# PaoPaoRobot/ygz-slam

Measured on NVIDIA H100. Metric: tracked frames/sec, higher is better.
Workload: dtype u8+f32+f64

## Files before the change

ygz_slam_b200/csrc/align.cu:

```cuda
#include <algorithm>
#include <cstdlib>
#include <mutex>

#include <cooperative_groups.h>

#include "common.cuh"
#include "se3.cuh"
#include "track.cuh"

namespace ygzb {

namespace {

struct LevelImg {
    const uint8_t* d;
    int w, h, pitch;
};

__device__ __forceinline__ LevelImg level_img(const uint8_t* pyr, size_t slot_stride, int slot, const Geometry& g, int L) {
    return LevelImg{pyr + (size_t)slot * slot_stride + g.lv[L].off, g.lv[L].w, g.lv[L].h, g.lv[L].pitch};
}

__device__ void inverse3f(const float H[3][3], float inv[3][3]) {
#define COF(i, j) (H[(i + 1) % 3][(j + 1) % 3] * H[(i + 2) % 3][(j + 2) % 3] - H[(i + 1) % 3][(j + 2) % 3] * H[(i + 2) % 3][(j + 1) % 3])
// ... 289 lines not shown
    const uint8_t* has_mp;
    const double* T_ref;
    double* T_cur;
    int max_level, min_level, n_iter;
    double eps;
    int32_t* n_meas_out;
    int32_t* iters_out;
    float* ref_patch;
    float* gdx;
    float* gdy;
    double* frame_jac;
    uint8_t* visible;
    double* ws;
    void* feat_scratch;
    size_t feat_stride;
};

constexpr int kSparseCluster = 8;
constexpr int kSparseThreads = 256;
constexpr int kNormalTerms = 21 + 6 + 1;

__device__ bool ldlt_solve6(const double H[6][6], const double b[6], double x[6]) {
    double L[6][6], D[6];
    for (int i = 0; i < 6; ++i)
        for (int j = 0; j < 6; ++j) L[i][j] = 0;
    for (int j = 0; j < 6; ++j) {
        double d = H[j][j];
        for (int k = 0; k < j; ++k) d -= L[j][k] * L[j][k] * D[k];
        D[j] = d;
        if (!(fabs(d) > 0)) return false;
// ... 202 lines not shown
        if (rank == 0 && tid == 0 && a.iters_out) a.iters_out[prob * kMaxLevels + lvl] = it;
        __syncthreads();
    }
    cluster.sync();
    if (rank == 0 && tid == 0) {
        const SE3d Tref = se3_from_mat(a.T_ref + 12 * (size_t)prob);
        se3_to_mat(se3_mul(s_T, Tref), a.T_cur + 12 * (size_t)prob);
        a.n_meas_out[prob] = (int32_t)(s_last_nmeas / 16);
    }
}


constexpr int kSA2Threads = 256;
constexpr int kSA2Terms = 21 + 6 + 1;

struct SA2Feat {
    float patch[16], gdx[16], gdy[16];
    double FJ[12];
    double G[3];
    double xyz[3];
    float u, v;
    int ui, vi;
    int state;
    int pad;
};

__device__ __forceinline__ double sa2_rcp(double x) {
    double r;
    asm("rcp.approx.ftz.f64 %0, %1;" : "=d"(r) : "d"(x));
    r = fma(r, fma(-x, r, 1.0), r);
    r = fma(r, fma(-x, r, 1.0), r);
    return r;
}

__device__ bool ldlt_solve6_fast(const double H[6][6], const double b[6], double x[6]) {
    double L[6][6], D[6], rD[6];
    for (int j = 0; j < 6; ++j) {
        double d = H[j][j];
        for (int k = 0; k < j; ++k) d -= L[j][k] * L[j][k] * D[k];
// ... 15 lines not shown
        y[i] = s;
    }
    for (int i = 0; i < 6; ++i) y[i] *= rD[i];
    for (int i = 5; i >= 0; --i) {
        double s = y[i];
        for (int k = i + 1; k < 6; ++k) s -= L[k][i] * x[k];
        x[i] = s;
    }
    return true;
}

__global__ void __launch_bounds__(kSA2Threads) sparse_align2_kernel(const SparseArgs a, int feat_cap ) {
    namespace cg = cooperative_groups;
    cg::cluster_group cluster = cg::this_cluster();
    extern __shared__ __align__(16) unsigned char s_raw[];
    __shared__ double s_red[kSA2Threads / 32][kSA2Terms];
    __shared__ unsigned s_nm[kSA2Threads / 32];
    __shared__ double s_part[2][kSA2Terms + 1];
    __shared__ SE3d s_T, s_old;
    __shared__ double s_Tm[12];
    __shared__ int s_flag;
    __shared__ double s_chi2;
    __shared__ unsigned long long s_last_nmeas;

    const int rank = (int)cluster.block_rank(), C = (int)cluster.num_blocks();
    const int prob = blockIdx.x / C, tid = threadIdx.x, lane = tid & 31, warp = tid >> 5;
    const int f0 = a.offsets[prob];
    const int nf = a.n_feat ? a.n_feat[prob] : a.offsets[prob + 1] - f0;
    const long din = a.in_off ? (long)a.in_off[prob] - f0 : 0;
    const Geometry& g = a.g;
    if (nf == 0) {
        if (rank == 0 && tid == 0) a.n_meas_out[prob] = 0;
        return;
    }
    const int per = (nf + C - 1) / C;
    const int j_lo = min(nf, rank * per), nl = min(nf, j_lo + per) - j_lo;
    SA2Feat* F = nl <= feat_cap ? reinterpret_cast<SA2Feat*>(s_raw)
                                : reinterpret_cast<SA2Feat*>(static_cast<unsigned char*>(a.feat_scratch) + (size_t)prob * a.feat_stride) + j_lo;
    if (tid == 0) {
        const SE3d Tref = se3_from_mat(a.T_ref + 12 * (size_t)prob);
        s_T = se3_mul(se3_from_mat(a.T_cur + 12 * (size_t)prob), se3_inverse(Tref));
        s_chi2 = 1e10;
        s_last_nmeas = 0;
    }
    for (int j = tid; j < nl; j += kSA2Threads) {
        SA2Feat& ft = F[j];
        const long gi = f0 + j_lo + j + din;
        ft.state = 0;
        const V3d xyz = pixel2camera(a.cam, a.px[2 * gi], a.px[2 * gi + 1], a.depth[gi]);
        ft.xyz[0] = xyz.x; ft.xyz[1] = xyz.y; ft.xyz[2] = xyz.z;
        for (int k = 0; k < 16; ++k) ft.patch[k] = 0.f;
    }
    __syncthreads();
    int slot = 0;

    for (int lvl = a.max_level; lvl >= a.min_level; --lvl) {
        const LevelImg rim = level_img(a.pyr, a.slot_stride, a.ref_slot[prob], g, lvl);
        const LevelImg cim = level_img(a.pyr, a.slot_stride, a.cur_slot[prob], g, lvl);
        const float scale = 1.0f / (float)(1 << lvl);
        const double focal = (double)(float)((a.cam.fx + a.cam.fy) / 2);
        const double jscale = focal / (1 << lvl);
        for (int j = tid; j < nl; j += kSA2Threads) {
            SA2Feat& ft = F[j];
            const long gi = f0 + j_lo + j + din;
            for (int k = 0; k < 16; ++k) ft.gdx[k] = ft.gdy[k] = 0.f;
            ft.G[0] = ft.G[1] = ft.G[2] = 0.0;
            const float u_ref = (float)(a.px[2 * gi] * scale), v_ref = (float)(a.px[2 * gi + 1] * scale);
            const int ui = (int)floorf(u_ref), vi = (int)floorf(v_ref);
            if ((a.has_mp && !a.has_mp[gi]) || ui - 3 < 0 || vi - 3 < 0 || ui + 3 >= rim.w || vi + 3 >= rim.h) continue;
            ft.state |= 1;
            const double X = ft.xyz[0], Y = ft.xyz[1], zi = 1. / ft.xyz[2], zi2 = zi * zi;
            double* J = ft.FJ;
            J[0] = -zi; J[1] = 0; J[2] = X * zi2; J[3] = Y * J[2]; J[4] = -(1.0 + X * J[2]); J[5] = Y * zi;
            J[6] = 0; J[7] = -zi; J[8] = Y * zi2; J[9] = 1.0 + Y * J[8]; J[10] = -J[3]; J[11] = -X * zi;
            const float su = u_ref - (float)ui, sv = v_ref - (float)vi;
            const float wtl = (float)((1.0 - su) * (1.0 - sv)), wtr = (float)(su * (1.0 - sv)), wbl = (float)((1.0 - su) * sv), wbr = su * sv;
            const int st = rim.pitch;
            int pc = 0;
            double gxx = 0, gxy = 0, gyy = 0;
// ... 2 lines not shown
                for (int xx = 0; xx < 4; ++xx, ++p, ++pc) {
                    ft.patch[pc] = wtl * (float)p[0] + wtr * (float)p[1] + wbl * (float)p[st] + wbr * (float)p[st + 1];
                    const float dx = 0.5f * ((wtl * (float)p[1] + wtr * (float)p[2] + wbl * (float)p[st + 1] + wbr * (float)p[st + 2]) -
                                             (wtl * (float)p[-1] + wtr * (float)p[0] + wbl * (float)p[st - 1] + wbr * (float)p[st]));
                    const float dy = 0.5f * ((wtl * (float)p[st] + wtr * (float)p[1 + st] + wbl * (float)p[st * 2] + wbr * (float)p[st * 2 + 1]) -
                                             (wtl * (float)p[-st] + wtr * (float)p[1 - st] + wbl * (float)p[0] + wbr * (float)p[1]));
                    ft.gdx[pc] = dx;
                    ft.gdy[pc] = dy;
                    gxx += (double)dx * (double)dx;
                    gxy += (double)dx * (double)dy;
                    gyy += (double)dy * (double)dy;
                }
            }
            ft.G[0] = gxx; ft.G[1] = gxy; ft.G[2] = gyy;
        }
        if (tid == 0) {
            s_old = s_T;
            s_flag = 0;
            se3_to_mat(s_T, s_Tm);
        }
        __syncthreads();

        int it = 0;
        for (it = 0; it < a.n_iter; ++it) {
            for (int j = tid; j < nl; j += kSA2Threads) {
                SA2Feat& ft = F[j];
                if (!(ft.state & 1)) continue;
                ft.state &= ~2;
                const double x = s_Tm[0] * ft.xyz[0] + s_Tm[1] * ft.xyz[1] + s_Tm[2] * ft.xyz[2] + s_Tm[3];
                const double y = s_Tm[4] * ft.xyz[0] + s_Tm[5] * ft.xyz[1] + s_Tm[6] * ft.xyz[2] + s_Tm[7];
                const double z = s_Tm[8] * ft.xyz[0] + s_Tm[9] * ft.xyz[1] + s_Tm[10] * ft.xyz[2] + s_Tm[11];
                double pu, pv;
                camera2pixel(a.cam, V3d{x, y, z}, &pu, &pv);
                const float u_cur = (float)pu * scale, v_cur = (float)pv * scale;
                const int ui = (int)floorf(u_cur), vi = (int)floorf(v_cur);
                if (ui < 0 || vi < 0 || ui - 3 < 0 || vi - 3 < 0 || ui + 3 >= cim.w || vi + 3 >= cim.h) continue;
                ft.u = u_cur; ft.v = v_cur; ft.ui = ui; ft.vi = vi;
                ft.state |= 2;
            }
            __syncthreads();
            double acc[kSA2Terms];
#pragma unroll
            for (int k = 0; k < kSA2Terms; ++k) acc[k] = 0.0;
            unsigned nm = 0;
            for (int item = tid; item < nl * 4; item += kSA2Threads) {
                const SA2Feat& ft = F[item >> 2];
                if ((ft.state & 3) != 3) continue;
                const int y = item & 3;
                const float su = ft.u - (float)ft.ui, sv = ft.v - (float)ft.vi;
                const float wtl = (float)((1.0 - su) * (1.0 - sv)), wtr = (float)(su * (1.0 - sv)), wbl = (float)((1.0 - su) * sv), wbr = su * sv;
                const int st = cim.pitch;
                const uint8_t* p = cim.d + (size_t)(ft.vi + y - 2) * st + (ft.ui - 2);
                double sa = 0, sb = 0;
#pragma unroll
                for (int xx = 0; xx < 4; ++xx, ++p) {
                    const int pc = 4 * y + xx;
                    const float inten = wtl * (float)p[0] + wtr * (float)p[1] + wbl * (float)p[st] + wbr * (float)p[st + 1];
                    const float res = inten - ft.patch[pc];
                    acc[27] += (double)(res * res);
                    sa += (double)ft.gdx[pc] * (double)res;
                    sb += (double)ft.gdy[pc] * (double)res;
                }
                nm += 4;
#pragma unroll
                for (int k = 0; k < 6; ++k) acc[21 + k] -= (ft.FJ[k] * sa + ft.FJ[6 + k] * sb) * jscale;
                if (y == 0) {
                    const double s2 = jscale * jscale, gxx = ft.G[0] * s2, gxy = ft.G[1] * s2, gyy = ft.G[2] * s2;
                    int t = 0;
#pragma unroll
                    for (int r = 0; r < 6; ++r)
#pragma unroll
                        for (int c = r; c < 6; ++c, ++t)
                            acc[t] += gxx * (ft.FJ[r] * ft.FJ[c]) + gxy * (ft.FJ[r] * ft.FJ[6 + c] + ft.FJ[6 + r] * ft.FJ[c]) + gyy * (ft.FJ[6 + r] * ft.FJ[6 + c]);
                }
            }
#pragma unroll
            for (int k = 0; k < kSA2Terms; ++k) {
                double v = acc[k];
#pragma unroll
                for (int o = 16; o > 0; o >>= 1) v += __shfl_down_sync(0xFFFFFFFFu, v, o);
                if (lane == 0) s_red[warp][k] = v;
            }
#pragma unroll
            for (int o = 16; o > 0; o >>= 1) nm += __shfl_down_sync(0xFFFFFFFFu, nm, o);
            if (lane == 0) s_nm[warp] = nm;
            __syncthreads();
            if (tid <= kSA2Terms) {
                double v = 0;
                if (tid < kSA2Terms) {
                    for (int w = 0; w < kSA2Threads / 32; ++w) v += s_red[w][tid];
                } else {
                    unsigned n = 0;
                    for (int w = 0; w < kSA2Threads / 32; ++w) n += s_nm[w];
                    v = (double)n;
                }
                s_part[slot][tid] = v;
            }
            cluster.sync();
            if (tid == 0) {
                double tot[kSA2Terms];
                unsigned long long n_meas = 0;
                for (int k = 0; k < kSA2Terms; ++k) tot[k] = 0;
                for (int r = 0; r < C; ++r) {
                    const double* pr = cluster.map_shared_rank(&s_part[slot][0], r);
                    for (int k = 0; k < kSA2Terms; ++k) tot[k] += pr[k];
                    n_meas += (unsigned long long)pr[kSA2Terms];
                }
                s_last_nmeas = n_meas;
                double H[6][6], b[6], x[6];
                int t = 0;
                for (int r = 0; r < 6; ++r)
                    for (int c = r; c < 6; ++c) H[r][c] = H[c][r] = tot[t++];
                for (int k = 0; k < 6; ++k) b[k] = tot[21 + k];
                const double new_chi2 = (double)((float)tot[27] / (float)n_meas);
                bool stop = !ldlt_solve6_fast(H, b, x) || isnan(x[0]);
                if ((it > 0 && new_chi2 > s_chi2) || stop) {
                    s_T = s_old;
                    s_flag = 1;
                } else {
                    double mx[6];
                    for (int k = 0; k < 6; ++k) mx[k] = -x[k];
                    const SE3d Tn = se3_mul(s_T, se3_exp(mx));
                    s_old = s_T;
                    s_T = Tn;
                    s_chi2 = new_chi2;
                    double nmx = -1;
                    for (int k = 0; k < 6; ++k) nmx = fabs(x[k]) > nmx ? fabs(x[k]) : nmx;
                    if (nmx <= a.eps) s_flag = 1;
                }
                se3_to_mat(s_T, s_Tm);
            }
            slot ^= 1;
            __syncthreads();
            if (s_flag) break;
        }
        if (rank == 0 && tid == 0 && a.iters_out) a.iters_out[prob * kMaxLevels + lvl] = it;
        __syncthreads();
    }
    cluster.sync();
    if (rank == 0 && tid == 0) {
        const SE3d Tref = se3_from_mat(a.T_ref + 12 * (size_t)prob);
        se3_to_mat(se3_mul(s_T, Tref), a.T_cur + 12 * (size_t)prob);
        a.n_meas_out[prob] = (int32_t)(s_last_nmeas / 16);
    }
}

__device__ __forceinline__ void mat34_mul(const double* A, const double* B, double* C) {
    for (int r = 0; r < 3; ++r) {
        for (int c = 0; c < 3; ++c) C[4 * r + c] = A[4 * r] * B[c] + A[4 * r + 1] * B[4 + c] + A[4 * r + 2] * B[8 + c];
        C[4 * r + 3] = A[4 * r] * B[3] + A[4 * r + 1] * B[7] + A[4 * r + 2] * B[11] + A[4 * r + 3];
    }
}
__device__ __forceinline__ void mat34_inv(const double* A, double* C) {
    for (int r = 0; r < 3; ++r) {
        for (int c = 0; c < 3; ++c) C[4 * r + c] = A[4 * c + r];
        C[4 * r + 3] = -(A[r] * A[3] + A[4 + r] * A[7] + A[8 + r] * A[11]);
    }
}
// ... 125 lines not shown
            b.c_px[2 * dst] = b.cand_px[2 * ((size_t)j * b.cap + c)];
            b.c_px[2 * dst + 1] = b.cand_px[2 * ((size_t)j * b.cap + c) + 1];
            b.c_pw[3 * dst] = st.kf_pw[3 * fe];
            b.c_pw[3 * dst + 1] = st.kf_pw[3 * fe + 1];
            b.c_pw[3 * dst + 2] = st.kf_pw[3 * fe + 2];
        }
        __syncthreads();
        if (tid == 0) s_carry += chunk_total;
        __syncthreads();
    }
    if (tid == 0) b.c_cnt[j] = s_carry;
}

}

size_t sparse_align2_scratch_bytes(int n_problems, int max_features) { return (size_t)n_problems * max_features * sizeof(SA2Feat); }
size_t sparse_align_ws_doubles(int n_problems) { return (size_t)n_problems * 2 * kSparseCluster * (kNormalTerms + 1); }

int launch_align2d(ygzb_frames* f, int n, const int32_t* d_slot, const uint8_t* d_level, const uint8_t* d_ref_border,
                   const uint8_t* d_ref, int n_iter, double* d_uv, uint8_t* d_ok) {
    ygzb_ctx* ctx = f->ctx;
    if (n <= 0) return YGZB_OK;
    ProfScope ps(ctx, kStageAlign2D);
    align2d_kernel<<<(n + 127) / 128, 128, 0, ctx->stream>>>(f->d_pyr, ctx->slot_stride, ctx->geo, n, d_slot, d_level, d_ref_border,
                                                             d_ref, n_iter, d_uv, d_ok);
    YGZB_LAUNCHED(ctx);
    return YGZB_OK;
}

int launch_align1d(ygzb_frames* f, int n, const int32_t* d_slot, const uint8_t* d_level, const float* d_dir, const uint8_t* d_ref_border,
                   const uint8_t* d_ref, int n_iter, double* d_uv, uint8_t* d_ok, double* d_hinv) {
// ... 29 lines not shown
    cfg.dynamicSmemBytes = 0;
    cfg.stream = ctx->stream;
    cudaLaunchAttribute attr[1];
    attr[0].id = cudaLaunchAttributeClusterDimension;
    attr[0].val.clusterDim.x = cluster;
    attr[0].val.clusterDim.y = 1;
    attr[0].val.clusterDim.z = 1;
    cfg.attrs = attr;
    cfg.numAttrs = 1;
    ProfScope ps(ctx, kStageSparseAlign);
    YGZB_CUDA(ctx, cudaLaunchKernelEx(&cfg, sparse_align_kernel, a));
    YGZB_LAUNCHED(ctx);
    return YGZB_OK;
}

int launch_sparse_align2(ygzb_ctx* ctx, SparseArgs a, int n_problems, int cluster, void* feat_scratch, size_t feat_stride) {
    static std::once_flag once;
    static int max_dyn = 0;
    std::call_once(once, [&] {
        int dev = 0, optin = 0;
        cudaGetDevice(&dev);
        cudaDeviceGetAttribute(&optin, cudaDevAttrMaxSharedMemoryPerBlockOptin, dev);
        max_dyn = optin - 8 * 1024;
        cudaFuncSetAttribute(sparse_align2_kernel, cudaFuncAttributeMaxDynamicSharedMemorySize, max_dyn);
    });
    const int max_features = (int)(feat_stride / sizeof(SA2Feat));
    const int feat_cap = std::min(max_dyn / (int)sizeof(SA2Feat), (max_features + cluster - 1) / cluster);
    a.feat_scratch = feat_scratch;
    a.feat_stride = feat_stride;
    cudaLaunchConfig_t cfg{};
    cfg.gridDim = dim3((unsigned)(n_problems * cluster));
    cfg.blockDim = dim3(kSA2Threads);
    cfg.dynamicSmemBytes = (size_t)feat_cap * sizeof(SA2Feat);
    cfg.stream = ctx->stream;
    cudaLaunchAttribute attr[1];
    attr[0].id = cudaLaunchAttributeClusterDimension;
    attr[0].val.clusterDim.x = cluster;
    attr[0].val.clusterDim.y = 1;
    attr[0].val.clusterDim.z = 1;
    cfg.attrs = attr;
    cfg.numAttrs = 1;
    ProfScope ps(ctx, kStageSparseAlign);
    YGZB_CUDA(ctx, cudaLaunchKernelEx(&cfg, sparse_align2_kernel, a, feat_cap));
    YGZB_LAUNCHED(ctx);
    return YGZB_OK;
}

}
// ... 24 lines not shown
    a.T_cur = d_T_cur;
    a.max_level = max_level;
    a.min_level = min_level;
    a.n_iter = n_iter;
    a.eps = eps;
    a.n_meas_out = d_n_meas;
    a.iters_out = d_iters;
    a.ref_patch = d_ref_patch;
    a.gdx = d_gdx;
    a.gdy = d_gdy;
    a.frame_jac = d_frame_jac;
    a.visible = d_visible;
    a.ws = d_ws;
    a.feat_scratch = nullptr;
    a.feat_stride = 0;
    if (sparse_align_gen1()) return launch_sparse_align1(ctx, a, n_problems, kSparseCluster);
    return launch_sparse_align2(ctx, a, n_problems, kTrackCluster, d_feat_scratch, feat_stride);
}


int launch_track_chain_front(ygzb_frames* f, const TrackStore& st, const TrackBatch& b, int sparse_cluster) {
    ygzb_ctx* ctx = f->ctx;
    if (b.J <= 0) return YGZB_OK;
    {
        ProfScope ps(ctx, kStageOther);
        track_prep_kernel<<<(b.J + 127) / 128, 128, 0, ctx->stream>>>(st, b);
        YGZB_LAUNCHED(ctx);
    }
    const bool gen1 = sparse_align_gen1();
    if (gen1)
        YGZB_CUDA(ctx, cudaMemsetAsync(b.ref_patch, 0, (size_t)b.J * st.cells * 16 * sizeof(float), ctx->stream));
    SparseArgs a;
// ... 13 lines not shown
    a.T_cur = b.T_cur;
    a.max_level = 2;
    a.min_level = 0;
    a.n_iter = 30;
    a.eps = 1e-6;
    a.n_meas_out = b.n_meas;
    a.iters_out = nullptr;
    a.ref_patch = b.ref_patch;
    a.gdx = b.gdx;
    a.gdy = b.gdy;
    a.frame_jac = b.frame_jac;
    a.visible = b.visible;
    a.ws = b.sparse_ws;
    a.feat_scratch = nullptr;
    a.feat_stride = 0;
    if (gen1) return launch_sparse_align1(ctx, a, b.J, sparse_cluster);
    return launch_sparse_align2(ctx, a, b.J, sparse_cluster, b.sa2_scratch, sparse_align2_scratch_bytes(1, st.cells));
}

int launch_track_chain_mid(ygzb_frames* f, const TrackStore& st, const TrackBatch& b) {
    ygzb_ctx* ctx = f->ctx;
    if (b.J <= 0) return YGZB_OK;
    {
        ProfScope ps(ctx, kStageOther);
        track_compose_kernel<<<(b.J + 63) / 64, 64, 0, ctx->stream>>>(st, b);
        YGZB_LAUNCHED(ctx);
    }
    {
        ProfScope ps(ctx, kStageOther);
        track_motion_kernel<<<(b.J + 63) / 64, 64, 0, ctx->stream>>>(st, b);
        YGZB_LAUNCHED(ctx);
    }
// ... 17 lines not shown
```

ygz_slam_b200/csrc/common.cuh:

```cuda
#pragma once

#include <cuda_runtime.h>
#include <stdint.h>
#include <stdio.h>
#include <string.h>

#include <vector>

#include "../../include/ygz_b200.h"

namespace ygzb {

constexpr int kMaxLevels = YGZB_MAX_LEVELS;

constexpr int kTileW = 80;
constexpr int kTileH = 40;

struct LevelGeom {
    int w, h, pitch;
    unsigned off;
};

struct Geometry {
    LevelGeom lv[kMaxLevels];
// ... 121 lines not shown
                   const uint8_t* d_ref, int n_iter, double* d_uv, uint8_t* d_ok);
int launch_align1d(ygzb_frames* f, int n, const int32_t* d_slot, const uint8_t* d_level, const float* d_dir, const uint8_t* d_ref_border,
                   const uint8_t* d_ref, int n_iter, double* d_uv, uint8_t* d_ok, double* d_hinv);
int launch_project_align(ygzb_frames* f, int n, const int32_t* d_ref_slot, const int32_t* d_cur_slot, const double* d_poses,
                         const int32_t* d_ref_pose, const int32_t* d_cur_pose, const double* d_ref_px, const double* d_ref_depth,
                         const uint8_t* d_ref_level, double* d_cur_px, uint8_t* d_search_level, uint8_t* d_ok);
int launch_sparse_align(ygzb_frames* f, int n_problems, const int32_t* d_ref_slot, const int32_t* d_cur_slot,
                        const int32_t* d_offsets, const double* d_px, const double* d_depth, const uint8_t* d_has_mp,
                        const double* d_T_ref, double* d_T_cur, int max_level, int min_level, int n_iter, double eps,
                        int32_t* d_n_meas, int32_t* d_iters, float* d_ref_patch, float* d_gdx, float* d_gdy, double* d_frame_jac,
                        uint8_t* d_visible, double* d_ws, void* d_feat_scratch, size_t feat_stride);
bool sparse_align_gen1();
size_t sparse_align_ws_doubles(int n_problems);
size_t sparse_align2_scratch_bytes(int n_problems, int max_features);
constexpr int kTrackCluster = 4;

struct Carver {
    uint8_t* base;
    size_t off = 0;
    explicit Carver(void* p) : base(static_cast<uint8_t*>(p)) {}
    template <typename T>
    T* take(size_t count) {
        off = (off + 255) & ~(size_t)255;
        T* r = base ? reinterpret_cast<T*>(base + off) : nullptr;
        off += count * sizeof(T);
        return r;
    }
    size_t bytes() const { return off + 256; }
};

// ... 40 lines not shown
```

ygz_slam_b200/csrc/track.cu:

```cuda
#include <algorithm>
#include <cstdlib>
#include <cstring>
#include <new>

#include "ba2.cuh"
#include "common.cuh"
#include "se3.cuh"
#include "track.cuh"

using namespace ygzb;

struct ygzb_tracker {
    ygzb_frames* f;
    ygzb_ctx* ctx;
    TrackStore st;
    TrackBatch b;
    int max_jobs;
    void* d_store;
    void* d_batch;
    double* d_depth;
    ygzb_track_job* h_jobs;
    ygzb_keyframe_job* h_kfjobs;
    ygzb_keyframe_job* d_kfjobs;
    ygzb_keyframe_result* d_kfres;
    cudaEvent_t staged;
    int last_J;
    void* d_ba;
    size_t ba_bytes;
    int pcap, ocap;
    cudaStream_t front;
    cudaEvent_t e_fill;
    cudaEvent_t e_front;
    cudaEvent_t e_up;
    cudaEvent_t e_main;
    int cluster;
    void* d_xfer;
};

namespace {

template <typename T>
int dalloc(ygzb_ctx* ctx, T** p, size_t count) {
    return check_cuda(ctx, cudaMalloc((void**)p, std::max(count, (size_t)1) * sizeof(T)), "cudaMalloc");
}

__device__ __forceinline__ void mat34_inv(const double* A, double* C) {
    for (int r = 0; r < 3; ++r) {
        for (int c = 0; c < 3; ++c) C[4 * r + c] = A[4 * c + r];
        C[4 * r + 3] = -(A[r] * A[3] + A[4 + r] * A[7] + A[8 + r] * A[11]);
    }
}
// ... 417 lines not shown
    *out = nullptr;
    ygzb_ctx* ctx = f->ctx;
    cudaSetDevice(ctx->device);
    if (ctx->geo.n_cells > 4096) return set_error(ctx, YGZB_ERR_CAPACITY, "tracker: %d grid cells (the BA assembly handles up to 4096)", ctx->geo.n_cells);
    ygzb_tracker* t = new (std::nothrow) ygzb_tracker();
    if (!t) return YGZB_ERR_INVALID;
    memset(t, 0, sizeof(*t));
    t->f = f;
    t->ctx = ctx;
    t->max_jobs = max_jobs;
    t->cluster = kTrackCluster;
    if (const char* e = getenv("YGZB_TRACK_CLUSTER")) {
        const int v = atoi(e);
        if (v == 1 || v == 2 || v == 4 || v == 8) t->cluster = v;
    }
    const Geometry& g = ctx->geo;
    const size_t S = (size_t)n_streams, R = YGZB_TRACK_RING, cells = (size_t)g.n_cells, E = S * R, cap = kTrackMaxLocal * cells;
    TrackStore& st = t->st;
    st.S = n_streams; st.R = (int)R; st.cells = (int)cells; st.W = g.W; st.H = g.H;
    st.fx = K[0]; st.fy = K[1]; st.cx = K[2]; st.cy = K[3];
    int rc = YGZB_OK;
    {
        Carver sz(nullptr);
        sz.take<double>(E * 12); sz.take<int32_t>(E); sz.take<int32_t>(E); sz.take<long long>(E); sz.take<double>(E * cells * 2);
        sz.take<uint8_t>(E * cells); sz.take<double>(E * cells); sz.take<double>(E * cells * 3); sz.take<int32_t>(E);
        sz.take<long long>(E * cap); sz.take<double>(E * cap * 2);
        rc = check_cuda(ctx, cudaMalloc(&t->d_store, sz.bytes()), "cudaMalloc(tracker store)");
        if (rc == YGZB_OK) rc = check_cuda(ctx, cudaMemsetAsync(t->d_store, 0, sz.bytes(), ctx->stream), "memset");
        if (rc == YGZB_OK) {
            Carver c(t->d_store);
            st.kf_T = c.take<double>(E * 12); st.kf_n = c.take<int32_t>(E); st.kf_slot = c.take<int32_t>(E); st.kf_mp0 = c.take<long long>(E);
            st.kf_px = c.take<double>(E * cells * 2); st.kf_level = c.take<uint8_t>(E * cells); st.kf_depth = c.take<double>(E * cells);
            st.kf_pw = c.take<double>(E * cells * 3); st.kf_nobs = c.take<int32_t>(E); st.kf_obs_id = c.take<long long>(E * cap);
            st.kf_obs_px = c.take<double>(E * cap * 2);
        }
    }
    if (rc == YGZB_OK) rc = dalloc(ctx, &t->d_depth, S * g.W * g.H);
    st.depth_map = t->d_depth;
    if (rc == YGZB_OK) {
        const size_t J = (size_t)max_jobs, F = J * cells, Cn = J * cap;
        TrackBatch& b = t->b;
        b.J = 0;
        b.cap = (int)cap;
        auto carve = [&](Carver& c) {
            b.jobs = c.take<ygzb_track_job>(J);
            b.ref_slot = c.take<int32_t>(J); b.cur_slot = c.take<int32_t>(J); b.offsets = c.take<int32_t>(J + 1); b.in_off = c.take<int32_t>(J);
            b.n_feat = c.take<int32_t>(J); b.n_meas = c.take<int32_t>(J);
            b.T_ref = c.take<double>(J * 12); b.T_cur = c.take<double>(J * 12); b.T_aligned = c.take<double>(J * 12);
            b.ref_patch = c.take<float>(F * 16); b.gdx = c.take<float>(F * 16); b.gdy = c.take<float>(F * 16);
            b.frame_jac = c.take<double>(F * 12); b.visible = c.take<uint8_t>(F);
            b.sparse_ws = c.take<double>(sparse_align_ws_doubles((int)J));
            b.sa2_scratch = c.take<double>(sparse_align2_scratch_bytes((int)J, (int)cells) / 8 + 1);
            b.aligned = c.take<int32_t>(J); b.rel = c.take<double>(J * kTrackMaxLocal * 12);
            b.cand_ok = c.take<uint8_t>(Cn); b.cand_px = c.take<double>(Cn * 2); b.n_cand = c.take<int32_t>(J);
            b.c_cnt = c.take<int32_t>(J); b.c_off = c.take<int32_t>(J + 1); b.c_src = c.take<int32_t>(Cn);
            b.c_pw = c.take<double>(Cn * 3); b.c_px = c.take<double>(Cn * 2); b.c_depth = c.take<double>(Cn);
            b.inlier = c.take<uint8_t>(Cn); b.enable = c.take<uint8_t>(Cn); b.n_inl = c.take<int32_t>(J);
            b.pose_ws = c.take<double>(pose_only_ws_doubles((int)J));
            b.results = c.take<ygzb_track_result>(J);
        };
        Carver sz(nullptr);
        carve(sz);
        rc = check_cuda(ctx, cudaMalloc(&t->d_batch, sz.bytes()), "cudaMalloc(tracker batch)");
        if (rc == YGZB_OK) rc = check_cuda(ctx, cudaMemsetAsync(t->d_batch, 0, sz.bytes(), ctx->stream), "memset");
        if (rc == YGZB_OK) {
            Carver c(t->d_batch);
            carve(c);
        }
    }
    if (rc == YGZB_OK) rc = check_cuda(ctx, cudaMallocHost((void**)&t->h_jobs, sizeof(ygzb_track_job) * (size_t)max_jobs), "cudaMallocHost");
    if (rc == YGZB_OK) rc = check_cuda(ctx, cudaMallocHost((void**)&t->h_kfjobs, sizeof(ygzb_keyframe_job) * S), "cudaMallocHost");
    if (rc == YGZB_OK) rc = dalloc(ctx, &t->d_kfjobs, S);
    if (rc == YGZB_OK) rc = dalloc(ctx, &t->d_kfres, S);
    if (rc == YGZB_OK) rc = check_cuda(ctx, cudaMemsetAsync(t->d_kfres, 0, sizeof(ygzb_keyframe_result) * S, ctx->stream), "memset");
    if (rc == YGZB_OK) rc = check_cuda(ctx, cudaEventCreateWithFlags(&t->staged, cudaEventDisableTiming), "cudaEventCreate");
    if (rc == YGZB_OK) rc = check_cuda(ctx, cudaStreamCreateWithFlags(&t->front, cudaStreamNonBlocking), "cudaStreamCreate");
    for (cudaEvent_t* e : {&t->e_fill, &t->e_front, &t->e_main, &t->e_up})
        if (rc == YGZB_OK) rc = check_cuda(ctx, cudaEventCreateWithFlags(e, cudaEventDisableTiming), "cudaEventCreate");
    if (rc == YGZB_OK) {
        rc = check_cuda(ctx, cudaEventRecord(t->e_fill, ctx->stream), "cudaEventRecord");
        if (rc == YGZB_OK) rc = check_cuda(ctx, cudaEventRecord(t->e_main, ctx->stream), "cudaEventRecord");
        if (rc == YGZB_OK) rc = check_cuda(ctx, cudaEventRecord(t->e_up, ctx->stream), "cudaEventRecord");
    }
    if (rc == YGZB_OK) {
        t->pcap = (int)(kTrackMaxLocal * cells + 1);
// ... 10 lines not shown
        ygzb_tracker_destroy(t);
        return rc;
    }
    *out = t;
    return YGZB_OK;
}

void ygzb_tracker_destroy(ygzb_tracker* t) {
    if (!t) return;
    cudaSetDevice(t->ctx->device);
    cudaStreamSynchronize(t->ctx->stream);
    if (t->d_store) cudaFree(t->d_store);
    if (t->d_batch) cudaFree(t->d_batch);
    if (t->d_depth) cudaFree(t->d_depth);
    if (t->h_jobs) cudaFreeHost(t->h_jobs);
    if (t->h_kfjobs) cudaFreeHost(t->h_kfjobs);
    if (t->d_kfjobs) cudaFree(t->d_kfjobs);
    if (t->d_kfres) cudaFree(t->d_kfres);
    if (t->d_ba) cudaFree(t->d_ba);
    if (t->d_xfer) cudaFree(t->d_xfer);
    if (t->staged) cudaEventDestroy(t->staged);
    if (t->front) {
        cudaStreamSynchronize(t->front);
        cudaStreamDestroy(t->front);
    }
    for (cudaEvent_t e : {t->e_fill, t->e_front, t->e_main, t->e_up})
        if (e) cudaEventDestroy(e);
    delete t;
}

// ... 25 lines not shown
    if (n_jobs == 0) return YGZB_OK;
    ygzb_ctx* ctx = t->ctx;
    cudaSetDevice(ctx->device);
    if (n_jobs > t->max_jobs) return set_error(ctx, YGZB_ERR_CAPACITY, "%d jobs exceed the tracker's max_jobs %d", n_jobs, t->max_jobs);
    for (int j = 0; j < n_jobs; ++j) {
        const ygzb_track_job& q = jobs[j];
        if (q.stream < 0 || q.stream >= t->st.S || q.cur_slot < 0 || q.cur_slot >= t->f->capacity || q.n_local < 1 || q.n_local > kTrackMaxLocal - 1)
            return set_error(ctx, YGZB_ERR_INVALID, "track job %d: stream / slot / n_local out of range", j);
        for (int k = 0; k < q.n_local; ++k)
            if (q.entry[k] < 0 || q.entry[k] >= YGZB_TRACK_RING) return set_error(ctx, YGZB_ERR_INVALID, "track job %d: ring entry out of range", j);
    }
    YGZB_CUDA(ctx, cudaEventSynchronize(t->staged));
    memcpy(t->h_jobs, jobs, sizeof(ygzb_track_job) * (size_t)n_jobs);
    TrackBatch b = t->b;
    b.J = n_jobs;
    t->last_J = n_jobs;
    const int cl = t->cluster;
    int rc;
    {
        cudaStream_t main = ctx->stream;
        YGZB_CUDA(ctx, cudaStreamWaitEvent(t->front, t->e_fill, 0));
        YGZB_CUDA(ctx, cudaStreamWaitEvent(t->front, t->e_main, 0));
        ctx->stream = t->front;
        cudaError_t ce = cudaMemcpyAsync(const_cast<ygzb_track_job*>(t->b.jobs), t->h_jobs, sizeof(ygzb_track_job) * (size_t)n_jobs,
                                         cudaMemcpyHostToDevice, ctx->stream);
        if (ce == cudaSuccess) ce = cudaEventRecord(t->staged, ctx->stream);
        rc = ce == cudaSuccess ? launch_track_chain_front(t->f, t->st, b, cl) : check_cuda(ctx, ce, "H2D(track jobs)");
        if (rc == YGZB_OK) rc = check_cuda(ctx, cudaEventRecord(t->e_front, ctx->stream), "cudaEventRecord");
        ctx->stream = main;
        if (rc != YGZB_OK) return rc;
        YGZB_CUDA(ctx, cudaStreamWaitEvent(ctx->stream, t->e_front, 0));
    }
    rc = launch_track_chain_mid(t->f, t->st, b);
    if (rc != YGZB_OK) return rc;
    rc = launch_pose_only_dev(ctx, n_jobs, b.c_off, b.c_cnt, b.c_pw, b.c_px, b.T_cur, b.inlier, b.c_depth, b.n_inl, b.enable, b.pose_ws, cl, b.cap);
    if (rc != YGZB_OK) return rc;
    {
        ProfScope ps(ctx, kStageOther);
        track_finish_kernel<<<(n_jobs + 63) / 64, 64, 0, ctx->stream>>>(b);
        YGZB_LAUNCHED(ctx);
// ... 242 lines not shown
```

ygz_slam_b200/csrc/track.cuh:

```cuda
#pragma once

#include <stdint.h>

#include "../../include/ygz_b200.h"

struct ygzb_frames;

namespace ygzb {

constexpr int kTrackMaxLocal = 4;

struct TrackStore {
    int S, R, cells, W, H;
    double fx, fy, cx, cy;
    double* kf_T;
    int32_t* kf_n;
    int32_t* kf_slot;
    long long* kf_mp0;
    double* kf_px;
    uint8_t* kf_level;
    double* kf_depth;
    double* kf_pw;
    int32_t* kf_nobs;
    long long* kf_obs_id;
// ... 1 lines not shown
    const double* depth_map;
};

struct TrackBatch {
    int J;
    int cap;
    const ygzb_track_job* jobs;
    int32_t *ref_slot, *cur_slot, *offsets, *in_off, *n_feat, *n_meas;
    double *T_ref, *T_cur;
    double* T_aligned;
    float *ref_patch, *gdx, *gdy;
    double* frame_jac;
    uint8_t* visible;
    double* sparse_ws;
    void* sa2_scratch;
    int32_t* aligned;
    double* rel;
    uint8_t* cand_ok;
    double* cand_px;
    int32_t* n_cand;
    int32_t *c_cnt, *c_off;
    int32_t* c_src;
    double *c_pw, *c_px, *c_depth;
    uint8_t *inlier, *enable;
    int32_t* n_inl;
    double* pose_ws;
    ygzb_track_result* results;
};

int launch_track_chain_front(ygzb_frames* f, const TrackStore& st, const TrackBatch& b, int sparse_cluster);
// ... 8 lines not shown
```

Baseline: 29200.

## Batch sparse-alignment jobs sharing a reference frame into one cluster group

Consecutive track jobs that share the same reference keyframe entry are grouped, up to a configurable size with a default of 2. Each group is solved by a single cluster that builds the reference patches, gradients and Jacobians once and runs per-frame Gauss-Newton state side by side. The feature struct is split into a shared reference part and a per-frame current-projection part. This cuts redundant reference-side work and the number of launched clusters, but the per-frame reductions run serially inside the block, shared-memory use grows, and a group keeps iterating until its slowest frame converges.

```diff
diff --git a/ygz_slam_b200/csrc/align.cu b/ygz_slam_b200/csrc/align.cu
--- a/ygz_slam_b200/csrc/align.cu
+++ b/ygz_slam_b200/csrc/align.cu
@@ -327,6 +327,7 @@
     double* ws;
     void* feat_scratch;
     size_t feat_stride;
+    const int32_t* groups;
 };
 
 constexpr int kSparseCluster = 8;
@@ -559,15 +560,17 @@
 constexpr int kSA2Threads = 256;
 constexpr int kSA2Terms = 21 + 6 + 1;
 
-struct SA2Feat {
+struct SA2Ref {
     float patch[16], gdx[16], gdy[16];
     double FJ[12];
     double G[3];
     double xyz[3];
+    int state;
+    int pad;
+};
+struct SA2Cur {
     float u, v;
     int ui, vi;
-    int state;
-    int pad;
 };
 
 __device__ __forceinline__ double sa2_rcp(double x) {
@@ -613,38 +616,53 @@
     namespace cg = cooperative_groups;
     cg::cluster_group cluster = cg::this_cluster();
     extern __shared__ __align__(16) unsigned char s_raw[];
-    __shared__ double s_red[kSA2Threads / 32][kSA2Terms];
-    __shared__ unsigned s_nm[kSA2Threads / 32];
-    __shared__ double s_part[2][kSA2Terms + 1];
-    __shared__ SE3d s_T, s_old;
-    __shared__ double s_Tm[12];
-    __shared__ int s_flag;
-    __shared__ double s_chi2;
-    __shared__ unsigned long long s_last_nmeas;
+    __shared__ double s_red[kSA2MaxGroup][kSA2Threads / 32][kSA2Terms];
+    __shared__ unsigned s_nm[kSA2MaxGroup][kSA2Threads / 32];
+    __shared__ double s_part[2][kSA2MaxGroup][kSA2Terms + 1];
+    __shared__ SE3d s_T[kSA2MaxGroup], s_old[kSA2MaxGroup];
+    __shared__ double s_Tm[kSA2MaxGroup][12];
+    __shared__ int s_flag[kSA2MaxGroup];
+    __shared__ int s_iters[kSA2MaxGroup];
+    __shared__ double s_chi2[kSA2MaxGroup];
+    __shared__ unsigned long long s_last_nmeas[kSA2MaxGroup];
 
     const int rank = (int)cluster.block_rank(), C = (int)cluster.num_blocks();
-    const int prob = blockIdx.x / C, tid = threadIdx.x, lane = tid & 31, warp = tid >> 5;
-    const int f0 = a.offsets[prob];
-    const int nf = a.n_feat ? a.n_feat[prob] : a.offsets[prob + 1] - f0;
-    const long din = a.in_off ? (long)a.in_off[prob] - f0 : 0;
+    const int grp = blockIdx.x / C, tid = threadIdx.x, lane = tid & 31, warp = tid >> 5;
+    const int p0 = a.groups ? a.groups[2 * grp] : grp, G = a.groups ? a.groups[2 * grp + 1] : 1;
+    const int f0 = a.offsets[p0];
+    const int nf = a.n_feat ? a.n_feat[p0] : a.offsets[p0 + 1] - f0;
+    const long in0 = a.in_off ? (long)a.in_off[p0] : f0;
     const Geometry& g = a.g;
     if (nf == 0) {
-        if (rank == 0 && tid == 0) a.n_meas_out[prob] = 0;
+        if (rank == 0 && tid < G) a.n_meas_out[p0 + tid] = 0;
         return;
     }
     const int per = (nf + C - 1) / C;
     const int j_lo = min(nf, rank * per), nl = min(nf, j_lo + per) - j_lo;
-    SA2Feat* F = nl <= feat_cap ? reinterpret_cast<SA2Feat*>(s_raw)
-                                : reinterpret_cast<SA2Feat*>(static_cast<unsigned char*>(a.feat_scratch) + (size_t)prob * a.feat_stride) + j_lo;
-    if (tid == 0) {
-        const SE3d Tref = se3_from_mat(a.T_ref + 12 * (size_t)prob);
-        s_T = se3_mul(se3_from_mat(a.T_cur + 12 * (size_t)prob), se3_inverse(Tref));
-        s_chi2 = 1e10;
-        s_last_nmeas = 0;
+    SA2Ref* F;
+    unsigned char* cur_base;
+    size_t cur_stride;
+    if (nl <= feat_cap) {
+        F = reinterpret_cast<SA2Ref*>(s_raw);
+        cur_base = s_raw + (size_t)nl * sizeof(SA2Ref);
+        cur_stride = (size_t)nl * sizeof(SA2Cur);
+    } else {
+        unsigned char* base = static_cast<unsigned char*>(a.feat_scratch) + (size_t)p0 * a.feat_stride;
+        const size_t max_f = a.feat_stride / (sizeof(SA2Ref) + sizeof(SA2Cur));
+        F = reinterpret_cast<SA2Ref*>(base) + j_lo;
+        cur_base = base + max_f * sizeof(SA2Ref) + (size_t)j_lo * sizeof(SA2Cur);
+        cur_stride = a.feat_stride;
+    }
+    auto CU = [&](int fr) { return reinterpret_cast<SA2Cur*>(cur_base + (size_t)fr * cur_stride); };
+    if (tid < G) {
+        const SE3d Tref = se3_from_mat(a.T_ref + 12 * (size_t)(p0 + tid));
+        s_T[tid] = se3_mul(se3_from_mat(a.T_cur + 12 * (size_t)(p0 + tid)), se3_inverse(Tref));
+        s_chi2[tid] = 1e10;
+        s_last_nmeas[tid] = 0;
     }
     for (int j = tid; j < nl; j += kSA2Threads) {
-        SA2Feat& ft = F[j];
-        const long gi = f0 + j_lo + j + din;
+        SA2Ref& ft = F[j];
+        const long gi = in0 + j_lo + j;
         ft.state = 0;
         const V3d xyz = pixel2camera(a.cam, a.px[2 * gi], a.px[2 * gi + 1], a.depth[gi]);
         ft.xyz[0] = xyz.x; ft.xyz[1] = xyz.y; ft.xyz[2] = xyz.z;
@@ -654,14 +672,13 @@
     int slot = 0;
 
     for (int lvl = a.max_level; lvl >= a.min_level; --lvl) {
-        const LevelImg rim = level_img(a.pyr, a.slot_stride, a.ref_slot[prob], g, lvl);
-        const LevelImg cim = level_img(a.pyr, a.slot_stride, a.cur_slot[prob], g, lvl);
+        const LevelImg rim = level_img(a.pyr, a.slot_stride, a.ref_slot[p0], g, lvl);
         const float scale = 1.0f / (float)(1 << lvl);
         const double focal = (double)(float)((a.cam.fx + a.cam.fy) / 2);
         const double jscale = focal / (1 << lvl);
         for (int j = tid; j < nl; j += kSA2Threads) {
-            SA2Feat& ft = F[j];
-            const long gi = f0 + j_lo + j + din;
+            SA2Ref& ft = F[j];
+            const long gi = in0 + j_lo + j;
             for (int k = 0; k < 16; ++k) ft.gdx[k] = ft.gdy[k] = 0.f;
             ft.G[0] = ft.G[1] = ft.G[2] = 0.0;
             const float u_ref = (float)(a.px[2 * gi] * scale), v_ref = (float)(a.px[2 * gi + 1] * scale);
@@ -694,99 +711,113 @@
             }
             ft.G[0] = gxx; ft.G[1] = gxy; ft.G[2] = gyy;
         }
-        if (tid == 0) {
-            s_old = s_T;
-            s_flag = 0;
-            se3_to_mat(s_T, s_Tm);
+        if (tid < G) {
+            s_old[tid] = s_T[tid];
+            s_flag[tid] = 0;
+            s_iters[tid] = a.n_iter;
+            se3_to_mat(s_T[tid], s_Tm[tid]);
         }
         __syncthreads();
 
-        int it = 0;
-        for (it = 0; it < a.n_iter; ++it) {
-            for (int j = tid; j < nl; j += kSA2Threads) {
-                SA2Feat& ft = F[j];
-                if (!(ft.state & 1)) continue;
-                ft.state &= ~2;
-                const double x = s_Tm[0] * ft.xyz[0] + s_Tm[1] * ft.xyz[1] + s_Tm[2] * ft.xyz[2] + s_Tm[3];
-                const double y = s_Tm[4] * ft.xyz[0] + s_Tm[5] * ft.xyz[1] + s_Tm[6] * ft.xyz[2] + s_Tm[7];
-                const double z = s_Tm[8] * ft.xyz[0] + s_Tm[9] * ft.xyz[1] + s_Tm[10] * ft.xyz[2] + s_Tm[11];
+        for (int it = 0; it < a.n_iter; ++it) {
+            for (int q = tid; q < G * nl; q += kSA2Threads) {
+                const int fr = q / nl, j = q - fr * nl;
+                const SA2Ref& ft = F[j];
+                if (s_flag[fr] || !(ft.state & 1)) continue;
+                SA2Cur& cu = CU(fr)[j];
+                const double* Tm = s_Tm[fr];
+                cu.ui = -1;
+                const double x = Tm[0] * ft.xyz[0] + Tm[1] * ft.xyz[1] + Tm[2] * ft.xyz[2] + Tm[3];
+                const double y = Tm[4] * ft.xyz[0] + Tm[5] * ft.xyz[1] + Tm[6] * ft.xyz[2] + Tm[7];
+                const double z = Tm[8] * ft.xyz[0] + Tm[9] * ft.xyz[1] + Tm[10] * ft.xyz[2] + Tm[11];
                 double pu, pv;
                 camera2pixel(a.cam, V3d{x, y, z}, &pu, &pv);
                 const float u_cur = (float)pu * scale, v_cur = (float)pv * scale;
                 const int ui = (int)floorf(u_cur), vi = (int)floorf(v_cur);
+                const LevelImg cim = level_img(a.pyr, a.slot_stride, a.cur_slot[p0 + fr], g, lvl);
                 if (ui < 0 || vi < 0 || ui - 3 < 0 || vi - 3 < 0 || ui + 3 >= cim.w || vi + 3 >= cim.h) continue;
-                ft.u = u_cur; ft.v = v_cur; ft.ui = ui; ft.vi = vi;
-                ft.state |= 2;
+                cu.u = u_cur; cu.v = v_cur; cu.ui = ui; cu.vi = vi;
             }
             __syncthreads();
-            double acc[kSA2Terms];
-#pragma unroll
-            for (int k = 0; k < kSA2Terms; ++k) acc[k] = 0.0;
-            unsigned nm = 0;
-            for (int item = tid; item < nl * 4; item += kSA2Threads) {
-                const SA2Feat& ft = F[item >> 2];
-                if ((ft.state & 3) != 3) continue;
-                const int y = item & 3;
-                const float su = ft.u - (float)ft.ui, sv = ft.v - (float)ft.vi;
-                const float wtl = (float)((1.0 - su) * (1.0 - sv)), wtr = (float)(su * (1.0 - sv)), wbl = (float)((1.0 - su) * sv), wbr = su * sv;
-                const int st = cim.pitch;
-                const uint8_t* p = cim.d + (size_t)(ft.vi + y - 2) * st + (ft.ui - 2);
-                double sa = 0, sb = 0;
-#pragma unroll
-                for (int xx = 0; xx < 4; ++xx, ++p) {
-                    const int pc = 4 * y + xx;
-                    const float inten = wtl * (float)p[0] + wtr * (float)p[1] + wbl * (float)p[st] + wbr * (float)p[st + 1];
-                    const float res = inten - ft.patch[pc];
-                    acc[27] += (double)(res * res);
-                    sa += (double)ft.gdx[pc] * (double)res;
-                    sb += (double)ft.gdy[pc] * (double)res;
+#pragma unroll 1
+            for (int fr = 0; fr < G; ++fr) {
+                if (s_flag[fr]) continue;
+                const LevelImg cim = level_img(a.pyr, a.slot_stride, a.cur_slot[p0 + fr], g, lvl);
+                const SA2Cur* cur = CU(fr);
+                double acc[kSA2Terms];
+#pragma unroll
+                for (int k = 0; k < kSA2Terms; ++k) acc[k] = 0.0;
+                unsigned nm = 0;
+                for (int item = tid; item < nl * 4; item += kSA2Threads) {
+                    const SA2Ref& ft = F[item >> 2];
+                    if (!(ft.state & 1)) continue;
+                    const SA2Cur cu = cur[item >> 2];
+                    if (cu.ui < 0) continue;
+                    const int y = item & 3;
+                    const float su = cu.u - (float)cu.ui, sv = cu.v - (float)cu.vi;
+                    const float wtl = (float)((1.0 - su) * (1.0 - sv)), wtr = (float)(su * (1.0 - sv)), wbl = (float)((1.0 - su) * sv), wbr = su * sv;
+                    const int st = cim.pitch;
+                    const uint8_t* p = cim.d + (size_t)(cu.vi + y - 2) * st + (cu.ui - 2);
+                    double sa = 0, sb = 0;
+#pragma unroll
+                    for (int xx = 0; xx < 4; ++xx, ++p) {
+                        const int pc = 4 * y + xx;
+                        const float inten = wtl * (float)p[0] + wtr * (float)p[1] + wbl * (float)p[st] + wbr * (float)p[st + 1];
+                        const float res = inten - ft.patch[pc];
+                        acc[27] += (double)(res * res);
+                        sa += (double)ft.gdx[pc] * (double)res;
+                        sb += (double)ft.gdy[pc] * (double)res;
+                    }
+                    nm += 4;
+#pragma unroll
+                    for (int k = 0; k < 6; ++k) acc[21 + k] -= (ft.FJ[k] * sa + ft.FJ[6 + k] * sb) * jscale;
+                    if (y == 0) {
+                        const double s2 = jscale * jscale, gxx = ft.G[0] * s2, gxy = ft.G[1] * s2, gyy = ft.G[2] * s2;
+                        int t = 0;
+#pragma unroll
+                        for (int r = 0; r < 6; ++r)
+#pragma unroll
+                            for (int c = r; c < 6; ++c, ++t)
+                                acc[t] += gxx * (ft.FJ[r] * ft.FJ[c]) + gxy * (ft.FJ[r] * ft.FJ[6 + c] + ft.FJ[6 + r] * ft.FJ[c]) + gyy * (ft.FJ[6 + r] * ft.FJ[6 + c]);
+                    }
                 }
-                nm += 4;
-#pragma unroll
-                for (int k = 0; k < 6; ++k) acc[21 + k] -= (ft.FJ[k] * sa + ft.FJ[6 + k] * sb) * jscale;
-                if (y == 0) {
-                    const double s2 = jscale * jscale, gxx = ft.G[0] * s2, gxy = ft.G[1] * s2, gyy = ft.G[2] * s2;
-                    int t = 0;
-#pragma unroll
-                    for (int r = 0; r < 6; ++r)
-#pragma unroll
-                        for (int c = r; c < 6; ++c, ++t)
-                            acc[t] += gxx * (ft.FJ[r] * ft.FJ[c]) + gxy * (ft.FJ[r] * ft.FJ[6 + c] + ft.FJ[6 + r] * ft.FJ[c]) + gyy * (ft.FJ[6 + r] * ft.FJ[6 + c]);
+#pragma unroll
+                for (int k = 0; k < kSA2Terms; ++k) {
+                    double v = acc[k];
+#pragma unroll
+                    for (int o = 16; o > 0; o >>= 1) v += __shfl_down_sync(0xFFFFFFFFu, v, o);
+                    if (lane == 0) s_red[fr][warp][k] = v;
                 }
+#pragma unroll
+                for (int o = 16; o > 0; o >>= 1) nm += __shfl_down_sync(0xFFFFFFFFu, nm, o);
+                if (lane == 0) s_nm[fr][warp] = nm;
             }
-#pragma unroll
-            for (int k = 0; k < kSA2Terms; ++k) {
-                double v = acc[k];
-#pragma unroll
-                for (int o = 16; o > 0; o >>= 1) v += __shfl_down_sync(0xFFFFFFFFu, v, o);
-                if (lane == 0) s_red[warp][k] = v;
-            }
-#pragma unroll
-            for (int o = 16; o > 0; o >>= 1) nm += __shfl_down_sync(0xFFFFFFFFu, nm, o);
-            if (lane == 0) s_nm[warp] = nm;
             __syncthreads();
-            if (tid <= kSA2Terms) {
+            for (int q = tid; q < G * (kSA2Terms + 1); q += kSA2Threads) {
+                const int fr = q / (kSA2Terms + 1), k = q - fr * (kSA2Terms + 1);
+                if (s_flag[fr]) continue;
                 double v = 0;
-                if (tid < kSA2Terms) {
-                    for (int w = 0; w < kSA2Threads / 32; ++w) v += s_red[w][tid];
+                if (k < kSA2Terms) {
+                    for (int w = 0; w < kSA2Threads / 32; ++w) v += s_red[fr][w][k];
                 } else {
                     unsigned n = 0;
-                    for (int w = 0; w < kSA2Threads / 32; ++w) n += s_nm[w];
+                    for (int w = 0; w < kSA2Threads / 32; ++w) n += s_nm[fr][w];
                     v = (double)n;
                 }
-                s_part[slot][tid] = v;
+                s_part[slot][fr][k] = v;
             }
             cluster.sync();
-            if (tid == 0) {
+            if (tid < G && !s_flag[tid]) {
+                const int fr = tid;
                 double tot[kSA2Terms];
                 unsigned long long n_meas = 0;
                 for (int k = 0; k < kSA2Terms; ++k) tot[k] = 0;
                 for (int r = 0; r < C; ++r) {
-                    const double* pr = cluster.map_shared_rank(&s_part[slot][0], r);
+                    const double* pr = cluster.map_shared_rank(&s_part[slot][fr][0], r);
                     for (int k = 0; k < kSA2Terms; ++k) tot[k] += pr[k];
                     n_meas += (unsigned long long)pr[kSA2Terms];
                 }
-                s_last_nmeas = n_meas;
+                s_last_nmeas[fr] = n_meas;
                 double H[6][6], b[6], x[6];
                 int t = 0;
                 for (int r = 0; r < 6; ++r)
@@ -794,34 +825,41 @@
                 for (int k = 0; k < 6; ++k) b[k] = tot[21 + k];
                 const double new_chi2 = (double)((float)tot[27] / (float)n_meas);
                 bool stop = !ldlt_solve6_fast(H, b, x) || isnan(x[0]);
-                if ((it > 0 && new_chi2 > s_chi2) || stop) {
-                    s_T = s_old;
-                    s_flag = 1;
+                bool done = false;
+                if ((it > 0 && new_chi2 > s_chi2[fr]) || stop) {
+                    s_T[fr] = s_old[fr];
+                    done = true;
                 } else {
                     double mx[6];
                     for (int k = 0; k < 6; ++k) mx[k] = -x[k];
-                    const SE3d Tn = se3_mul(s_T, se3_exp(mx));
-                    s_old = s_T;
-                    s_T = Tn;
-                    s_chi2 = new_chi2;
+                    const SE3d Tn = se3_mul(s_T[fr], se3_exp(mx));
+                    s_old[fr] = s_T[fr];
+                    s_T[fr] = Tn;
+                    s_chi2[fr] = new_chi2;
                     double nmx = -1;
                     for (int k = 0; k < 6; ++k) nmx = fabs(x[k]) > nmx ? fabs(x[k]) : nmx;
-                    if (nmx <= a.eps) s_flag = 1;
+                    if (nmx <= a.eps) done = true;
                 }
-                se3_to_mat(s_T, s_Tm);
+                se3_to_mat(s_T[fr], s_Tm[fr]);
+                if (done) {
+                    s_flag[fr] = 1;
+                    s_iters[fr] = it;
+                }
             }
             slot ^= 1;
             __syncthreads();
-            if (s_flag) break;
-        }
-        if (rank == 0 && tid == 0 && a.iters_out) a.iters_out[prob * kMaxLevels + lvl] = it;
+            int active = 0;
+            for (int fr = 0; fr < G; ++fr) active |= !s_flag[fr];
+            if (!active) break;
+        }
+        if (rank == 0 && tid < G && a.iters_out) a.iters_out[(p0 + tid) * kMaxLevels + lvl] = s_iters[tid];
         __syncthreads();
     }
     cluster.sync();
-    if (rank == 0 && tid == 0) {
-        const SE3d Tref = se3_from_mat(a.T_ref + 12 * (size_t)prob);
-        se3_to_mat(se3_mul(s_T, Tref), a.T_cur + 12 * (size_t)prob);
-        a.n_meas_out[prob] = (int32_t)(s_last_nmeas / 16);
+    if (rank == 0 && tid < G) {
+        const SE3d Tref = se3_from_mat(a.T_ref + 12 * (size_t)(p0 + tid));
+        se3_to_mat(se3_mul(s_T[tid], Tref), a.T_cur + 12 * (size_t)(p0 + tid));
+        a.n_meas_out[p0 + tid] = (int32_t)(s_last_nmeas[tid] / 16);
     }
 }
 
@@ -977,7 +1015,9 @@
 
 }
 
-size_t sparse_align2_scratch_bytes(int n_problems, int max_features) { return (size_t)n_problems * max_features * sizeof(SA2Feat); }
+size_t sparse_align2_scratch_bytes(int n_problems, int max_features) {
+    return (size_t)n_problems * max_features * (sizeof(SA2Ref) + sizeof(SA2Cur));
+}
 size_t sparse_align_ws_doubles(int n_problems) { return (size_t)n_problems * 2 * kSparseCluster * (kNormalTerms + 1); }
 
 int launch_align2d(ygzb_frames* f, int n, const int32_t* d_slot, const uint8_t* d_level, const uint8_t* d_ref_border,
@@ -1037,24 +1077,28 @@
     return YGZB_OK;
 }
 
-int launch_sparse_align2(ygzb_ctx* ctx, SparseArgs a, int n_problems, int cluster, void* feat_scratch, size_t feat_stride) {
+int launch_sparse_align2(ygzb_ctx* ctx, SparseArgs a, int n_groups, int group_max, int cluster, void* feat_scratch, size_t feat_stride) {
     static std::once_flag once;
     static int max_dyn = 0;
     std::call_once(once, [&] {
         int dev = 0, optin = 0;
         cudaGetDevice(&dev);
         cudaDeviceGetAttribute(&optin, cudaDevAttrMaxSharedMemoryPerBlockOptin, dev);
-        max_dyn = optin - 8 * 1024;
+        cudaFuncAttributes fa{};
+        cudaFuncGetAttributes(&fa, sparse_align2_kernel);
+        max_dyn = optin - (int)fa.sharedSizeBytes;
         cudaFuncSetAttribute(sparse_align2_kernel, cudaFuncAttributeMaxDynamicSharedMemorySize, max_dyn);
     });
-    const int max_features = (int)(feat_stride / sizeof(SA2Feat));
-    const int feat_cap = std::min(max_dyn / (int)sizeof(SA2Feat), (max_features + cluster - 1) / cluster);
+    if (group_max < 1 || group_max > kSA2MaxGroup) return set_error(ctx, YGZB_ERR_INVALID, "sparse alignment: %d frames per group", group_max);
+    const int feat_bytes = (int)(sizeof(SA2Ref) + (size_t)group_max * sizeof(SA2Cur));
+    const int max_features = (int)(feat_stride / (sizeof(SA2Ref) + sizeof(SA2Cur)));
+    const int feat_cap = std::min(max_dyn / feat_bytes, (max_features + cluster - 1) / cluster);
     a.feat_scratch = feat_scratch;
     a.feat_stride = feat_stride;
     cudaLaunchConfig_t cfg{};
-    cfg.gridDim = dim3((unsigned)(n_problems * cluster));
+    cfg.gridDim = dim3((unsigned)(n_groups * cluster));
     cfg.blockDim = dim3(kSA2Threads);
-    cfg.dynamicSmemBytes = (size_t)feat_cap * sizeof(SA2Feat);
+    cfg.dynamicSmemBytes = (size_t)feat_cap * feat_bytes;
     cfg.stream = ctx->stream;
     cudaLaunchAttribute attr[1];
     attr[0].id = cudaLaunchAttributeClusterDimension;
@@ -1109,8 +1153,9 @@
     a.ws = d_ws;
     a.feat_scratch = nullptr;
     a.feat_stride = 0;
+    a.groups = nullptr;
     if (sparse_align_gen1()) return launch_sparse_align1(ctx, a, n_problems, kSparseCluster);
-    return launch_sparse_align2(ctx, a, n_problems, kTrackCluster, d_feat_scratch, feat_stride);
+    return launch_sparse_align2(ctx, a, n_problems, 1, kTrackCluster, d_feat_scratch, feat_stride);
 }
 
 
@@ -1154,8 +1199,9 @@
     a.ws = b.sparse_ws;
     a.feat_scratch = nullptr;
     a.feat_stride = 0;
+    a.groups = b.groups;
     if (gen1) return launch_sparse_align1(ctx, a, b.J, sparse_cluster);
-    return launch_sparse_align2(ctx, a, b.J, sparse_cluster, b.sa2_scratch, sparse_align2_scratch_bytes(1, st.cells));
+    return launch_sparse_align2(ctx, a, b.n_groups, b.group_max, sparse_cluster, b.sa2_scratch, sparse_align2_scratch_bytes(1, st.cells));
 }
 
 int launch_track_chain_mid(ygzb_frames* f, const TrackStore& st, const TrackBatch& b) {
diff --git a/ygz_slam_b200/csrc/common.cuh b/ygz_slam_b200/csrc/common.cuh
--- a/ygz_slam_b200/csrc/common.cuh
+++ b/ygz_slam_b200/csrc/common.cuh
@@ -159,6 +159,7 @@
 size_t sparse_align_ws_doubles(int n_problems);
 size_t sparse_align2_scratch_bytes(int n_problems, int max_features);
 constexpr int kTrackCluster = 4;
+constexpr int kSA2MaxGroup = 8;
 
 struct Carver {
     uint8_t* base;
diff --git a/ygz_slam_b200/csrc/track.cu b/ygz_slam_b200/csrc/track.cu
--- a/ygz_slam_b200/csrc/track.cu
+++ b/ygz_slam_b200/csrc/track.cu
@@ -35,6 +35,8 @@
     cudaEvent_t e_main;
     int cluster;
     void* d_xfer;
+    int sparse_group;
+    int32_t* h_groups;
 };
 
 namespace {
@@ -482,6 +484,11 @@
         const int v = atoi(e);
         if (v == 1 || v == 2 || v == 4 || v == 8) t->cluster = v;
     }
+    t->sparse_group = 2;
+    if (const char* e = getenv("YGZB_SPARSE_GROUP")) {
+        const int v = atoi(e);
+        if (v >= 1 && v <= kSA2MaxGroup) t->sparse_group = v;
+    }
     const Geometry& g = ctx->geo;
     const size_t S = (size_t)n_streams, R = YGZB_TRACK_RING, cells = (size_t)g.n_cells, E = S * R, cap = kTrackMaxLocal * cells;
     TrackStore& st = t->st;
@@ -512,6 +519,7 @@
         b.cap = (int)cap;
         auto carve = [&](Carver& c) {
             b.jobs = c.take<ygzb_track_job>(J);
+            b.groups = c.take<int32_t>(J * 2);
             b.ref_slot = c.take<int32_t>(J); b.cur_slot = c.take<int32_t>(J); b.offsets = c.take<int32_t>(J + 1); b.in_off = c.take<int32_t>(J);
             b.n_feat = c.take<int32_t>(J); b.n_meas = c.take<int32_t>(J);
             b.T_ref = c.take<double>(J * 12); b.T_cur = c.take<double>(J * 12); b.T_aligned = c.take<double>(J * 12);
@@ -537,6 +545,7 @@
         }
     }
     if (rc == YGZB_OK) rc = check_cuda(ctx, cudaMallocHost((void**)&t->h_jobs, sizeof(ygzb_track_job) * (size_t)max_jobs), "cudaMallocHost");
+    if (rc == YGZB_OK) rc = check_cuda(ctx, cudaMallocHost((void**)&t->h_groups, sizeof(int32_t) * 2 * (size_t)max_jobs), "cudaMallocHost");
     if (rc == YGZB_OK) rc = check_cuda(ctx, cudaMallocHost((void**)&t->h_kfjobs, sizeof(ygzb_keyframe_job) * S), "cudaMallocHost");
     if (rc == YGZB_OK) rc = dalloc(ctx, &t->d_kfjobs, S);
     if (rc == YGZB_OK) rc = dalloc(ctx, &t->d_kfres, S);
@@ -577,6 +586,7 @@
     if (t->d_batch) cudaFree(t->d_batch);
     if (t->d_depth) cudaFree(t->d_depth);
     if (t->h_jobs) cudaFreeHost(t->h_jobs);
+    if (t->h_groups) cudaFreeHost(t->h_groups);
     if (t->h_kfjobs) cudaFreeHost(t->h_kfjobs);
     if (t->d_kfjobs) cudaFree(t->d_kfjobs);
     if (t->d_kfres) cudaFree(t->d_kfres);
@@ -632,6 +642,21 @@
     memcpy(t->h_jobs, jobs, sizeof(ygzb_track_job) * (size_t)n_jobs);
     TrackBatch b = t->b;
     b.J = n_jobs;
+    b.n_groups = 0;
+    b.group_max = 0;
+    for (int j = 0, e_prev = -1; j < n_jobs; ++j) {
+        const int e = jobs[j].stream * t->st.R + jobs[j].entry[jobs[j].n_local - 1];
+        int32_t* last = t->h_groups + 2 * (b.n_groups - 1);
+        if (b.n_groups && e == e_prev && last[1] < t->sparse_group) {
+            ++last[1];
+        } else {
+            t->h_groups[2 * b.n_groups] = j;
+            t->h_groups[2 * b.n_groups + 1] = 1;
+            ++b.n_groups;
+        }
+        b.group_max = std::max(b.group_max, t->h_groups[2 * b.n_groups - 1]);
+        e_prev = e;
+    }
     t->last_J = n_jobs;
     const int cl = t->cluster;
     int rc;
@@ -642,6 +667,8 @@
         ctx->stream = t->front;
         cudaError_t ce = cudaMemcpyAsync(const_cast<ygzb_track_job*>(t->b.jobs), t->h_jobs, sizeof(ygzb_track_job) * (size_t)n_jobs,
                                          cudaMemcpyHostToDevice, ctx->stream);
+        if (ce == cudaSuccess)
+            ce = cudaMemcpyAsync(b.groups, t->h_groups, sizeof(int32_t) * 2 * (size_t)b.n_groups, cudaMemcpyHostToDevice, ctx->stream);
         if (ce == cudaSuccess) ce = cudaEventRecord(t->staged, ctx->stream);
         rc = ce == cudaSuccess ? launch_track_chain_front(t->f, t->st, b, cl) : check_cuda(ctx, ce, "H2D(track jobs)");
         if (rc == YGZB_OK) rc = check_cuda(ctx, cudaEventRecord(t->e_front, ctx->stream), "cudaEventRecord");
diff --git a/ygz_slam_b200/csrc/track.cuh b/ygz_slam_b200/csrc/track.cuh
--- a/ygz_slam_b200/csrc/track.cuh
+++ b/ygz_slam_b200/csrc/track.cuh
@@ -39,6 +39,8 @@
     uint8_t* visible;
     double* sparse_ws;
     void* sa2_scratch;
+    int32_t* groups;
+    int n_groups, group_max;
     int32_t* aligned;
     double* rel;
     uint8_t* cand_ok;
```

After: 29540, median of 6. Within noise of the previous version (+1.2%).
